# kurtosis/mat_mul

Hardware: NVIDIA B200
Metric: env_steps_per_sec (higher is better)
Workload: dtype int8

## Files before the change

mat_mul_b200/csrc/tg_demo.cu:

```cuda
#include <cstring>
#include <mutex>

#include "tg_demo_mma.cuh"
#include "tg_demo_sampler.cuh"
#include "tg_step.cuh"

namespace tg {

template <int S, int NT, int NPASS = 1>
struct DemoCfg {
    using G = Geo<S>;
    static constexpr int GPASS = NT / S;
    static constexpr int TG = GPASS * NPASS;
    static constexpr int ACTIVE = GPASS * S;
    static constexpr bool TILE = S != 4;
    static constexpr int KW = (S + 3) / 4;
    static constexpr int NCW = (2 * S + 3) / 4;
    static constexpr int NW = (3 * S + 3) / 4;
    static constexpr int REC = G::TP;
    static_assert(4 * (KW + NCW) <= REC, "record does not fit the token pitch");
    static constexpr int PITCH = G::GP + (S == 9 ? 32 : (S == 4 ? 16 : 0));
    static constexpr int PASS_SLAB = TILE ? GPASS * PITCH : 0;
    static __host__ __device__ constexpr int rec_bytes(int R) { return R * TG * REC; }
    static __host__ __device__ constexpr int rec_region(int R) { return (rec_bytes(R) + 15) & ~15; }
    static constexpr bool SPLIT = S == 9;
    static constexpr int REC_SMEM = SPLIT ? 36 : REC;
    static __host__ __device__ constexpr int pass_rec(int R) { return GPASS * R * REC_SMEM; }
    static __host__ __device__ constexpr int pass_stride(int R) { return ((pass_rec(R) > PASS_SLAB ? pass_rec(R) : PASS_SLAB) + 15) & ~15; }
    static __host__ __device__ constexpr int main_bytes(int R) { return NPASS * pass_stride(R); }
    static __device__ __forceinline__ void rec_pos(int g, int r, int R, int &region, int &k) {
        const int pass = NPASS == 1 ? 0 : g / GPASS;
        region = pass * pass_stride(R), k = (g - pass * GPASS) * R + r;
    }
    static __device__ __forceinline__ int slab_off(int g, int R) {
        if constexpr (NPASS == 1) return g * PITCH;
        const int pass = g / GPASS;
        return pass * pass_stride(R) + (g - pass * GPASS) * PITCH;
    }
    static constexpr int FLAG_BYTES = ((TG + 3) & ~3) * 4;
    static __host__ __device__ constexpr int smem_bytes(int R) { return main_bytes(R) + FLAG_BYTES + 16 + 2 * NT * 4; }
};

template <int S, int NT, int NPASS, bool SMALL>
__device__ __forceinline__ void emit_record(const uint32_t words[(3 * S + 3) / 4], int shift, uint8_t *region, int k, int R) {
    using C = DemoCfg<S, NT, NPASS>;
    constexpr int o = 2 * S;
    constexpr uint32_t WLAST = (S % 4) ? (0xFFFFFFFFu >> (8 * (4 - S % 4))) : 0xFFFFFFFFu;
    const uint32_t sh4 = (uint32_t)shift * ONES4;
    uint32_t out[C::REC / 4];
#pragma unroll
    for (int m = 0; m < C::REC / 4; m++) out[m] = 0;
#pragma unroll
    for (int m = 0; m < C::KW; m++) {
        const uint32_t lo = words[(o >> 2) + m];
        uint32_t wt = lo;
        if constexpr ((o & 3) != 0) {
            const uint32_t hi = ((o >> 2) + m + 1 < C::NW) ? words[(o >> 2) + m + 1] : 0u;
            wt = __funnelshift_r(lo, hi, 8 * (o & 3));
        }
        const uint32_t msk = (m == C::KW - 1) ? WLAST : 0xFFFFFFFFu;
        out[m] = (wt & msk) - (sh4 & msk);
    }
#pragma unroll
    for (int m = 0; m < C::NCW; m++) out[C::KW + m] = SMALL ? (words[m] + (H4 - sh4)) ^ H4 : ((words[m] | H4) - sh4) ^ H4;
    if constexpr (C::SPLIT) {
        static_assert(!C::SPLIT || (C::KW == 3 && C::NCW == 5), "split records: 9x9x9");
        const int n = C::GPASS * R;
        *reinterpret_cast<uint4 *>(region + k * 16) = make_uint4(out[0], out[1], out[2], out[3]);
        *reinterpret_cast<uint2 *>(region + n * 16 + k * 8) = make_uint2(out[4], out[5]);
        uint32_t *v = reinterpret_cast<uint32_t *>(region + n * 24 + k * 12);
        v[0] = out[5], v[1] = out[6], v[2] = out[7];
    } else {
        static_assert(C::REC % 16 == 0, "record pitch");
        uint8_t *rec = region + k * C::REC;
#pragma unroll
        for (int m = 0; m < C::REC / 16; m++)
            reinterpret_cast<uint4 *>(rec)[m] = make_uint4(out[4 * m], out[4 * m + 1], out[4 * m + 2], out[4 * m + 3]);
    }
}

template <int B>
__device__ __forceinline__ int coef_byte(uint32_t w) {
    constexpr uint32_t sel = (uint32_t)B | ((uint32_t)(B | 8) << 4) | ((uint32_t)(B | 8) << 8) | ((uint32_t)(B | 8) << 12);
    return (int)prmt(w, 0u, sel);
}

template <int S, int NT, int NPASS, bool SAMPLE, int NTHR, bool GUARD, int MMA = 0, bool ALIAS = false>
__global__ void __launch_bounds__(NT, S == 16 ? (NT <= 128 ? 4 : 2) : (S == 9 ? (NT == 128 ? 8 : NT == 64 ? 16 : 3) : 4))
    demo_kernel(unsigned long long first_demo, long long N, int R, uint32_t magic_r, int shift,
                const __grid_constant__ Categorical cat, int max_tries, uint8_t *__restrict__ tape,
                long long tape_step_stride, int8_t *__restrict__ slab, uint8_t *__restrict__ flags,
                const __grid_constant__ AliasDev ap) {
    using C = DemoCfg<S, NT, NPASS>;
    using G = Geo<S>;
    extern __shared__ __align__(128) uint8_t smem[];
    uint8_t *s_rec = smem;
    constexpr int MMA_SCRATCH = MMA > 0 ? (NT / 32) * acc16::WARP_WORDS * 4 : 0;
    uint32_t *s_flag = reinterpret_cast<uint32_t *>(smem + (MMA == 0 ? C::main_bytes(R) : MMA > 0 ? C::rec_region(R) + MMA_SCRATCH : 0));
    uint32_t *s_work = s_flag + C::FLAG_BYTES / 4;
    uint32_t *s_list = s_work + 4;
    uint32_t *s_alias = MMA > 0 ? reinterpret_cast<uint32_t *>(smem + C::rec_region(R)) : s_list;

    const int tid = threadIdx.x;
    const int lane = tid & 31;
    const long long g0 = (long long)blockIdx.x * C::TG;
    const int ng = (int)min((long long)C::TG, N - g0);
    const int npairs = ng * R;

    for (int g = tid; g < C::TG; g += NT) s_flag[g] = 0;
    if (tid < 3) s_work[tid] = 0;
    if constexpr (ALIAS) alias_to_smem<S, NT>(ap, s_alias);
    __syncthreads();

    if constexpr (SAMPLE && ALIAS) {
        for (int p = tid; p < npairs; p += NT) {
            const int g = magic_r ? (int)__umulhi((uint32_t)p, magic_r) : p;
            const int r = p - g * R;
            const unsigned long long d = first_demo + (unsigned long long)(g0 + g);
            uint32_t words[G::TP / 4];
#pragma unroll
            for (int w = C::NW; w < G::TP / 4; w++) words[w] = 0;
            draw_triple_alias<S>(words, (uint32_t)d, (uint32_t)(d >> 32), r, ap, s_alias);
            uint4 *dst = reinterpret_cast<uint4 *>(tape + (size_t)r * tape_step_stride + (g0 + g) * G::TP);
#pragma unroll
            for (int w = 0; w < G::TP / 16; w++) dst[w] = make_uint4(words[4 * w], words[4 * w + 1], words[4 * w + 2], words[4 * w + 3]);
            if constexpr (MMA == 0) {
                {
                    int region, k;
                    C::rec_pos(g, r, R, region, k);
                    emit_record<S, NT, NPASS, true>(words, shift, smem + region, k, R);
                }
            } else if constexpr (MMA > 0) {
                uint4 *rdst = reinterpret_cast<uint4 *>(s_rec + ((size_t)g * R + r) * G::TP);
#pragma unroll
                for (int w = 0; w < G::TP / 16; w++) rdst[w] = make_uint4(words[4 * w], words[4 * w + 1], words[4 * w + 2], words[4 * w + 3]);
            }
        }
    } else if constexpr (SAMPLE) {
        auto decode = [&](int p, int &g, int &r, uint32_t &d_lo, uint32_t &d_hi) {
            g = magic_r ? (int)__umulhi((uint32_t)p, magic_r) : p;
            r = p - g * R;
            const unsigned long long d = first_demo + (unsigned long long)(g0 + g);
            d_lo = (uint32_t)d, d_hi = (uint32_t)(d >> 32);
        };
        auto attempt = [&](int g, int r, uint32_t d_lo, uint32_t d_hi, int t) -> bool {
            uint32_t words[G::TP / 4];
#pragma unroll
            for (int w = C::NW; w < G::TP / 4; w++) words[w] = 0;
            bool ok = draw_triple<S, NTHR>(words, d_lo, d_hi, r, t, cat);
            if (!ok && t + 1 >= max_tries) {
#pragma unroll
                for (int w = 0; w < C::NW; w++) words[w] = 0;
#pragma unroll
                for (int q = 0; q < 3 * S; q++)
                    words[q >> 2] |= (((q % S) == 0 ? cat.top_tok : (uint32_t)shift) & 0xFFu) << (8 * (q & 3));
                atomicOr(&s_flag[g], (uint32_t)TG_FLAG_EXHAUSTED);
                ok = true;
            }
            if (ok) {
                uint4 *dst = reinterpret_cast<uint4 *>(tape + (size_t)r * tape_step_stride + (g0 + g) * G::TP);
#pragma unroll
                for (int w = 0; w < G::TP / 16; w++)
                    dst[w] = make_uint4(words[4 * w], words[4 * w + 1], words[4 * w + 2], words[4 * w + 3]);
                if constexpr (MMA == 0) {
                    {
                    int region, k;
                    C::rec_pos(g, r, R, region, k);
                    emit_record<S, NT, NPASS, false>(words, shift, smem + region, k, R);
                }
                } else if constexpr (MMA > 0) {
                    uint4 *rdst = reinterpret_cast<uint4 *>(s_rec + ((size_t)g * R + r) * G::TP);
#pragma unroll
                    for (int w = 0; w < G::TP / 16; w++)
                        rdst[w] = make_uint4(words[4 * w], words[4 * w + 1], words[4 * w + 2], words[4 * w + 3]);
                }
            }
            return ok;
        };
        auto park = [&](bool pending, int p, int t, int which) {
            const uint32_t m = __ballot_sync(0xFFFFFFFFu, pending);
            if (m) {
                const int leader = __ffs(m) - 1;
                int base = 0;
                if (lane == leader) base = (int)atomicAdd(&s_work[1 + which], (uint32_t)__popc(m));
                base = __shfl_sync(0xFFFFFFFFu, base, leader);
                if (pending) s_list[which * NT + base + __popc(m & ((1u << lane) - 1u))] = (uint32_t)p | ((uint32_t)t << 16);
            }
        };
        {
            int p = npairs, t = 0, g = 0, r = 0;
            uint32_t d_lo = 0, d_hi = 0;
            bool need = true;
            while (true) {
                const uint32_t m = __ballot_sync(0xFFFFFFFFu, need);
                if (m) {
                    const int leader = __ffs(m) - 1;
                    int base = 0;
                    if (lane == leader) base = (int)atomicAdd(&s_work[0], (uint32_t)__popc(m));
                    base = __shfl_sync(0xFFFFFFFFu, base, leader);
                    if (need) {
                        p = base + __popc(m & ((1u << lane) - 1u));
                        t = 0, need = false;
                        if (p < npairs) decode(p, g, r, d_lo, d_hi);
                    }
                }
                if (__ballot_sync(0xFFFFFFFFu, p >= npairs) != 0) {
                    park(p < npairs, p, t, 0);
                    break;
                }
                if (attempt(g, r, d_lo, d_hi, t))
                    need = true;
                else
                    t++;
            }
        }
        __syncthreads();
        for (int cur = 0;; cur ^= 1) {
            const int n = (int)s_work[1 + cur];
            if (n == 0) break;
            __syncthreads();
            if (tid == 0) s_work[1 + (cur ^ 1)] = 0;
            __syncthreads();
            const bool have = tid < n;
            int p = 0, t = 0, g = 0, r = 0;
            uint32_t d_lo = 0, d_hi = 0;
            bool pending = false;
            if (have) {
                const uint32_t it = s_list[cur * NT + tid];
                p = (int)(it & 0xFFFFu), t = (int)(it >> 16);
                decode(p, g, r, d_lo, d_hi);
                pending = true;
            }
#pragma unroll 1
            for (int k = 0; k < 3; k++) {
                if (pending) {
                    pending = !attempt(g, r, d_lo, d_hi, t);
                    t++;
                }
                if (__ballot_sync(0xFFFFFFFFu, pending) == 0) break;
            }
            park(pending, p, t, cur ^ 1);
            __syncthreads();
        }
    } else {
        for (int p = tid; p < npairs; p += NT) {
            const int g = magic_r ? (int)__umulhi((uint32_t)p, magic_r) : p;
            const int r = p - g * R;
            const uint4 *src = reinterpret_cast<const uint4 *>(tape + (size_t)r * tape_step_stride + (g0 + g) * G::TP);
            uint32_t words[G::TP / 4];
#pragma unroll
            for (int w = 0; w < G::TP / 16; w++) {
                const uint4 q = src[w];
                words[4 * w] = q.x, words[4 * w + 1] = q.y, words[4 * w + 2] = q.z, words[4 * w + 3] = q.w;
            }
            {
                    int region, k;
                    C::rec_pos(g, r, R, region, k);
                    emit_record<S, NT, NPASS, false>(words, shift, smem + region, k, R);
                }
        }
    }
    __syncthreads();
    if constexpr (MMA != 0) {
        if constexpr (MMA > 0) {
            static_assert(MMA <= 0 || (S == 16 && G::TP == 48), "tensor-core accumulation: 16x16x16 only");
            const int warp = tid >> 5;
            uint32_t *sH = reinterpret_cast<uint32_t *>(smem + C::rec_region(R)) + warp * acc16::WARP_WORDS, *sU = sH + acc16::H_WORDS;
            for (int g = warp; g < ng; g += NT / 32) {
#pragma unroll
                for (int pass = 0; pass < (MMA + 1) / 2; pass++) {
                    const int r = 32 * pass + lane;
                    if (r < 16 * MMA) {
                        const uint32_t z = (uint32_t)shift * ONES4;
                        uint4 raw[3] = {make_uint4(z, z, z, z), make_uint4(z, z, z, z), make_uint4(z, z, z, z)};
                        if (r < R) {
                            const uint4 *src = reinterpret_cast<const uint4 *>(s_rec + ((size_t)g * R + r) * G::TP);
                            raw[0] = src[0], raw[1] = src[1], raw[2] = src[2];
                        }
                        acc16::record_to_halves(raw, shift, sH + r * acc16::HP);
                    }
                }
                __syncwarp();
                const bool bad = acc16::gemms_from_halves<MMA>(sH, sU, slab + (g0 + g) * G::GP, lane);
                if (bad && lane == 0) s_flag[g] |= (uint32_t)TG_FLAG_RANGE;
            }
            __syncthreads();
        }
        if (flags)
            for (int gg = tid; gg < ng; gg += NT) flags[g0 + gg] = (uint8_t)s_flag[gg];
        return;
    }

    constexpr int KW = C::KW;
    const bool sparse = cat.sparse_terms && R <= 32;
#pragma unroll 1
    for (int pass = 0; pass < NPASS; pass++) {
    int gl = tid / S, j = tid % S;
    bool worker = tid < C::ACTIVE && pass * C::GPASS + gl < ng;
    uint32_t tmask = 0;
    if (sparse) {
        if (worker) {
            const uint8_t *region = smem + pass * C::pass_stride(R);
            const int8_t *vb = reinterpret_cast<const int8_t *>(
                C::SPLIT ? region + C::GPASS * R * 24 + gl * R * 12 + 1 + j : region + gl * R * C::REC + 4 * C::KW + S + j);
            uint32_t bit = 1;
#pragma unroll 4
            for (int r = 0; r < R; r++, bit <<= 1)
                if (vb[r * (C::SPLIT ? 12 : C::REC)] != 0) tmask |= bit;
        }
    }
    const int g = pass * C::GPASS + gl;
// ... 243 lines not shown
    }
    const int warp = threadIdx.x >> 5, lane = threadIdx.x & 31;
    const long long nw0 = (long long)blockIdx.x * 128 + warp * 32;
    if (nw0 >= N) return;
    const bool real = nw0 + lane < N;
    const long long n = min(nw0 + lane, N - 1);
    const unsigned long long d = first_demo + (unsigned long long)n;
    uint32_t acc[16];
#pragma unroll
    for (int e = 0; e < 16; e++) acc[e] = H4;
    const uint32_t sh4 = (uint32_t)shift * ONES4;
    uint4 *rec = reinterpret_cast<uint4 *>(tape + n * 16);
    const long long stride16 = tape_step_stride / 16;
    uint4 nextq = (!SAMPLE && R > 0) ? __ldg(reinterpret_cast<const uint4 *>(rec)) : make_uint4(0, 0, 0, 0);
    for (int r = 0; r < R; r++) {
        uint32_t words[3];
        uint32_t cu, cv;
        if constexpr (SAMPLE) {
            draw_triple_alias<S>(words, (uint32_t)d, (uint32_t)(d >> 32), r, ap, s_alias);
            if (real) rec[(long long)r * stride16] = make_uint4(words[0], words[1], words[2], 0u);
            cu = (words[0] + (H4 - sh4)) ^ H4, cv = (words[1] + (H4 - sh4)) ^ H4;
        } else {
            words[0] = nextq.x, words[1] = nextq.y, words[2] = nextq.z;
            if (r + 1 < R) nextq = __ldg(reinterpret_cast<const uint4 *>(rec) + (long long)(r + 1) * stride16);
            cu = ((words[0] | H4) - sh4) ^ H4, cv = ((words[1] | H4) - sh4) ^ H4;
        }
        const int wi = (int)(words[2] - sh4);
        const int vw[4] = {coef_byte<0>(cv) * wi, coef_byte<1>(cv) * wi, coef_byte<2>(cv) * wi, coef_byte<3>(cv) * wi};
        const int u[4] = {coef_byte<0>(cu), coef_byte<1>(cu), coef_byte<2>(cu), coef_byte<3>(cu)};
#pragma unroll
        for (int i = 0; i < 4; i++)
#pragma unroll
            for (int j = 0; j < 4; j++) acc[4 * i + j] += (uint32_t)(u[i] * vw[j]);
    }
    uint32_t ok = H4;
    uint4 *mine = reinterpret_cast<uint4 *>(s_stage[warp] + lane * PITCH);
#pragma unroll
    for (int i = 0; i < 4; i++) {
#pragma unroll
        for (int j = 0; j < 4; j++) {
            const uint32_t o = acc[4 * i + j];
            ok &= o ^ (o << 1);
            acc[4 * i + j] = o ^ H4;
        }
        mine[i] = make_uint4(acc[4 * i], acc[4 * i + 1], acc[4 * i + 2], acc[4 * i + 3]);
    }
    if (flags && real) flags[n] = (~ok & H4) ? (uint8_t)TG_FLAG_RANGE : (uint8_t)0;
    __syncwarp();
    const int total = (int)min(32LL, N - nw0) * 4;
    uint4 *out = reinterpret_cast<uint4 *>(slab + nw0 * 64);
    for (int x = lane; x < total; x += 32) out[x] = *reinterpret_cast<const uint4 *>(s_stage[warp] + (x >> 2) * PITCH + (x & 3) * 16);
}

static int dispatch_demo_alias(unsigned long long first, long long N, int R, int S, int shift, const Categorical &cat,
                               const AliasDev &ap, uint8_t *tape, long long stride, int8_t *slab, uint8_t *flags, cudaStream_t st) {
    switch (S) {
    case 4:
#ifdef TG_TUNING
        if (tuning_env("TG_DEMO_VARIANT", 0) == 0)
#endif
        if ((long long)R * shift * shift * shift <= 191 && R <= 65535) {
            const long long grid = (N + 127) / 128;
            if (grid > 0x7FFFFFFFLL) return TG_E_ARG;
            demo4_thread_kernel<true><<<(int)grid, 128, 0, st>>>(first, N, R, shift, tape, stride, slab, flags, ap);
            TG_CUDA(cudaGetLastError());
            return TG_OK;
        }
        if (DemoCfg<4, 256, 4>::smem_bytes(R) <= 160 * 1024)
            return launch_demo_alias<4, 256, 4, 0>(first, N, R, shift, cat, ap, tape, stride, slab, flags, st);
        return launch_demo_alias<4, 256, 1, 0>(first, N, R, shift, cat, ap, tape, stride, slab, flags, st);
    case 9:
#ifdef TG_TUNING
        switch (tuning_env("TG_DEMO_VARIANT", 0)) {
        case 1: return launch_demo_alias<9, 256, 1, 0>(first, N, R, shift, cat, ap, tape, stride, slab, flags, st);
        case 2: return launch_demo_alias<9, 128, 1, 0>(first, N, R, shift, cat, ap, tape, stride, slab, flags, st);
        case 3: return launch_demo_alias<9, 256, 2, 0>(first, N, R, shift, cat, ap, tape, stride, slab, flags, st);
        case 4: return launch_demo_alias<9, 64, 2, 0>(first, N, R, shift, cat, ap, tape, stride, slab, flags, st);
        case 5: return launch_demo_alias<9, 64, 1, 0>(first, N, R, shift, cat, ap, tape, stride, slab, flags, st);
        default: break;
        }
#endif
        return launch_demo_alias<9, 128, 2, 0>(first, N, R, shift, cat, ap, tape, stride, slab, flags, st);
    case 16:
        if (demo_acc16_mma_applies(R)) {
            if (R <= 32) return launch_demo_alias<16, 128, 2, 2>(first, N, R, shift, cat, ap, tape, stride, slab, flags, st);
            return launch_demo_alias<16, 128, 2, 4>(first, N, R, shift, cat, ap, tape, stride, slab, flags, st);
        }
        return launch_demo_alias<16, 128, 1, 0>(first, N, R, shift, cat, ap, tape, stride, slab, flags, st);
    }
    return TG_E_ARG;
}

constexpr int ALIAS_SLOTS = 8, ALIAS_MAXDEV = 64;
__device__ __align__(16) uint32_t g_alias_tab[ALIAS_SLOTS][8 * ALIAS_BUCKETS];
__global__ void alias_upload_kernel(const __grid_constant__ AliasTabs t, int slot) {
    for (int w = threadIdx.x; w < 8 * ALIAS_BUCKETS; w += blockDim.x) g_alias_tab[slot][w] = (&t.tab[0][0])[w];
}
struct AliasSlot {
    bool valid = false;
    AliasTabs host;
    cudaEvent_t ready = nullptr;
    unsigned long long stamp = 0;
};
static AliasSlot g_alias_slots[ALIAS_MAXDEV][ALIAS_SLOTS];
static std::mutex g_alias_mu;
static unsigned long long g_alias_stamp = 0;

int alias_device_tables(const AliasTabs &want, cudaStream_t st, const uint32_t **dptr) {
    int dev = 0;
    TG_CUDA(cudaGetDevice(&dev));
    if (dev < 0 || dev >= ALIAS_MAXDEV) return TG_E_ARG;
    uint32_t *base = nullptr;
    TG_CUDA(cudaGetSymbolAddress(reinterpret_cast<void **>(&base), g_alias_tab));
    std::lock_guard<std::mutex> lock(g_alias_mu);
    AliasSlot *slots = g_alias_slots[dev];
    int hit = -1, lru = -1;
    for (int i = 0; i < ALIAS_SLOTS; i++) {
        if (slots[i].valid && memcmp(&slots[i].host, &want, sizeof(AliasTabs)) == 0) hit = i;
        if (lru < 0 || (slots[lru].valid && (!slots[i].valid || slots[i].stamp < slots[lru].stamp))) lru = i;
    }
    if (hit < 0) {
        AliasSlot &sl = slots[lru];
        if (sl.valid) TG_CUDA(cudaDeviceSynchronize());
        if (!sl.ready) TG_CUDA(cudaEventCreateWithFlags(&sl.ready, cudaEventDisableTiming));
        sl.valid = false;
        alias_upload_kernel<<<1, 256, 0, st>>>(want, lru);
        TG_CUDA(cudaGetLastError());
        TG_CUDA(cudaEventRecord(sl.ready, st));
        sl.host = want, sl.valid = true;
        hit = lru;
    } else {
        TG_CUDA(cudaStreamWaitEvent(st, slots[hit].ready, 0));
    }
    slots[hit].stamp = ++g_alias_stamp;
    *dptr = base + (size_t)hit * 8 * ALIAS_BUCKETS;
// ... 76 lines not shown
    }
    __syncthreads();
    if (flags && tid == 0) flags[n] = (uint8_t)((or_flags ? flags[n] : 0) | s_bad);
}

template <int S>
static int launch_demo_acc_cols(const uint8_t *tape, long long stride, long long N, int R, int shift, int8_t *slab, uint8_t *flags,
                                int or_flags, cudaStream_t st) {
    const long long smem = (long long)R * Geo<S>::TP;
    if (smem > 227 * 1024 || N > 0x7FFFFFFFLL) return TG_E_ARG;
    auto kern = demo_acc_cols_kernel<S>;
    TG_CUDA(cudaFuncSetAttribute(kern, cudaFuncAttributeMaxDynamicSharedMemorySize, (int)smem));
    kern<<<(unsigned)N, 160, (size_t)smem, st>>>(tape, stride, N, R, shift, slab, flags, or_flags);
    TG_CUDA(cudaGetLastError());
    return TG_OK;
}

template <int NTHR>
static int launch_demo25(unsigned long long first, long long N, int R, int shift, const Categorical &cat, int max_tries, uint8_t *tape,
                         long long stride, int8_t *slab, uint8_t *flags, cudaStream_t st) {
    constexpr int NT = 128;
    using C = DemoCfg<25, NT, 1>;
    const int smem = C::FLAG_BYTES + 16 + 2 * NT * 4;
    if (R > 65535 || (long long)C::TG * R >= (1LL << 16)) return TG_E_ARG;
    const uint32_t magic = R == 1 ? 0u : (uint32_t)((0x100000000ULL + (unsigned)R - 1) / (unsigned)R);
    const long long grid = (N + C::TG - 1) / C::TG;
    if (grid > 0x7FFFFFFFLL) return TG_E_ARG;
    static const AliasDev no_alias = {};
    demo_kernel<25, NT, 1, true, NTHR, false, -1><<<(int)grid, NT, smem, st>>>(first, N, R, magic, shift, cat, max_tries, tape, stride,
                                                                              nullptr, flags, no_alias);
    TG_CUDA(cudaGetLastError());
    return launch_demo_acc_cols<25>(tape, stride, N, R, shift, slab, flags, 1, st);
}

template <bool SAMPLE, int NTHR>
static int dispatch_demo(unsigned long long first, long long N, int R, int S, int shift, const Categorical &cat,
                         int max_tries, uint8_t *tape, long long stride, int8_t *slab, uint8_t *flags, cudaStream_t st) {
    switch (S) {
    case 4: {
#ifdef TG_TUNING
        static const int variant = tuning_env("TG_DEMO_VARIANT", 0);
        if (variant == 1 && DemoCfg<4, 128, 8>::smem_bytes(R) <= 160 * 1024)
            return launch_demo<4, 128, 8, SAMPLE, NTHR>(first, N, R, shift, cat, max_tries, tape, stride, slab, flags, st);
        if (variant == 2 && DemoCfg<4, 128, 4>::smem_bytes(R) <= 160 * 1024)
            return launch_demo<4, 128, 4, SAMPLE, NTHR>(first, N, R, shift, cat, max_tries, tape, stride, slab, flags, st);
        if (variant == 3 && DemoCfg<4, 512, 2>::smem_bytes(R) <= 160 * 1024)
            return launch_demo<4, 512, 2, SAMPLE, NTHR>(first, N, R, shift, cat, max_tries, tape, stride, slab, flags, st);
#endif
        if (DemoCfg<4, 256, 4>::smem_bytes(R) <= 160 * 1024)
            return launch_demo<4, 256, 4, SAMPLE, NTHR>(first, N, R, shift, cat, max_tries, tape, stride, slab, flags, st);
        return launch_demo<4, 256, 1, SAMPLE, NTHR>(first, N, R, shift, cat, max_tries, tape, stride, slab, flags, st);
    }
    case 9: {
#ifdef TG_TUNING
        switch (tuning_env("TG_DEMO_VARIANT", 0)) {
        case 1: return launch_demo<9, 256, 1, SAMPLE, NTHR>(first, N, R, shift, cat, max_tries, tape, stride, slab, flags, st);
        case 3: return launch_demo<9, 128, 3, SAMPLE, NTHR>(first, N, R, shift, cat, max_tries, tape, stride, slab, flags, st);
        case 4: return launch_demo<9, 192, 2, SAMPLE, NTHR>(first, N, R, shift, cat, max_tries, tape, stride, slab, flags, st);
        case 5: return launch_demo<9, 64, 4, SAMPLE, NTHR>(first, N, R, shift, cat, max_tries, tape, stride, slab, flags, st);
        default: break;
        }
#endif
        if (SAMPLE) return launch_demo<9, 128, 2, SAMPLE, NTHR>(first, N, R, shift, cat, max_tries, tape, stride, slab, flags, st);
        return launch_demo<9, 128, 1, SAMPLE, NTHR>(first, N, R, shift, cat, max_tries, tape, stride, slab, flags, st);
    }
    case 16: {
#ifdef TG_TUNING
        static const int variant = tuning_env("TG_DEMO_VARIANT", 0);
        if (variant == 1) return launch_demo<16, 256, 1, SAMPLE, NTHR>(first, N, R, shift, cat, max_tries, tape, stride, slab, flags, st);
        if (variant == 2) return launch_demo<16, 64, 1, SAMPLE, NTHR>(first, N, R, shift, cat, max_tries, tape, stride, slab, flags, st);
        if (variant == 3) return launch_demo<16, 128, 2, SAMPLE, NTHR>(first, N, R, shift, cat, max_tries, tape, stride, slab, flags, st);
#endif
        return launch_demo<16, 128, 1, SAMPLE, NTHR>(first, N, R, shift, cat, max_tries, tape, stride, slab, flags, st);
    }
    }
    return TG_E_ARG;
}

}

extern "C" {

int tg_demo_gen_philox(uint64_t seed, uint64_t first_demo, int64_t N, int R, int S, int shift, const int8_t *values,
                       const double *probs, int n_values, int max_tries, uint8_t *tape, int64_t tape_step_stride,
                       int8_t *slab, uint8_t *flags, void *stream) {
    if (!tg::supported_S(S) || N < 0 || R < 1 || shift < 1 || shift > 4 || n_values < 1 || n_values > 8 || max_tries < 1 ||
        max_tries > 65535)
        return TG_E_ARG;
    if (N == 0) return TG_OK;
    if (!values || !probs || !tape || !slab) return TG_E_ARG;
    if (((uintptr_t)tape | (uintptr_t)slab | (uintptr_t)tape_step_stride) & 15) return TG_E_ARG;
    if (!tg::alphabet_ok(values, probs, n_values, shift)) return TG_E_ARG;
    tg::Categorical cat = tg::categorical(values, probs, n_values, shift, seed);
    cat.sparse_terms = (S == 9 && tg::p_null<false>(values, probs, n_values) >= 0.5) ? 1u : 0u;
    cudaStream_t st = (cudaStream_t)stream;
    if (tg::alias_applies(values, probs, n_values, S)) {
        tg::AliasParams ap;
        tg::build_alias(values, probs, n_values, S, shift, seed, ap);
        tg::AliasTabs tabs;
        tg::AliasDev dev;
        tg::alias_to_dev(ap, values, n_values, S, shift, tabs, dev);
        const int rc = tg::alias_device_tables(tabs, st, &dev.tab);
        if (rc != TG_OK) return rc;
        return tg::dispatch_demo_alias(first_demo, N, R, S, shift, cat, dev, tape, tape_step_stride, slab, flags, st);
    }
#ifdef TG_TUNING
    static const int use_mma = tg::tuning_env("TG_DEMO_MMA", 1);
#else
    constexpr int use_mma = 1;
#endif
    if (S == 25) {
        if (n_values <= 3) return tg::launch_demo25<2>(first_demo, N, R, shift, cat, max_tries, tape, tape_step_stride, slab, flags, st);
        if (n_values <= 5) return tg::launch_demo25<4>(first_demo, N, R, shift, cat, max_tries, tape, tape_step_stride, slab, flags, st);
        return tg::launch_demo25<7>(first_demo, N, R, shift, cat, max_tries, tape, tape_step_stride, slab, flags, st);
    }
    if (S == 16 && use_mma && tg::demo_acc16_mma_applies(R)) {
        if (n_values <= 3) return tg::dispatch_demo16_mma<2>(first_demo, N, R, shift, cat, max_tries, tape, tape_step_stride, slab, flags, st);
        if (n_values <= 5) return tg::dispatch_demo16_mma<4>(first_demo, N, R, shift, cat, max_tries, tape, tape_step_stride, slab, flags, st);
        return tg::dispatch_demo16_mma<7>(first_demo, N, R, shift, cat, max_tries, tape, tape_step_stride, slab, flags, st);
    }
    if (n_values <= 3)
        return tg::dispatch_demo<true, 2>(first_demo, N, R, S, shift, cat, max_tries, tape, tape_step_stride, slab, flags, st);
    if (n_values <= 5)
        return tg::dispatch_demo<true, 4>(first_demo, N, R, S, shift, cat, max_tries, tape, tape_step_stride, slab, flags, st);
    return tg::dispatch_demo<true, 7>(first_demo, N, R, S, shift, cat, max_tries, tape, tape_step_stride, slab, flags, st);
}

int tg_demo_alias_tables(const int8_t *values, const double *probs, int n_values, int S, uint16_t *tables_host) {
    if (!values || !probs || !tables_host || !tg::alias_applies(values, probs, n_values, S)) return TG_E_ARG;
    tg::AliasParams ap;
    tg::build_alias(values, probs, n_values, S, 0, 0, ap);
    memcpy(tables_host, ap.tab[6], sizeof(ap.tab[6]));
    memcpy(tables_host + tg::ALIAS_BUCKETS, ap.tab[7], sizeof(ap.tab[7]));
    memcpy(tables_host + 2 * tg::ALIAS_BUCKETS, ap.tab[0], 6 * sizeof(ap.tab[0]));
    return TG_OK;
}

int tg_demo_accumulate(const uint8_t *tape, int64_t tape_step_stride, int64_t N, int R, int S, int shift, int8_t *slab,
                       uint8_t *flags, void *stream) {
    if (!tg::supported_S(S) || N < 0 || R < 1 || shift < 1 || shift > 4) return TG_E_ARG;
    if (N == 0) return TG_OK;
    if (!tape || !slab) return TG_E_ARG;
    if (((uintptr_t)tape | (uintptr_t)slab | (uintptr_t)tape_step_stride) & 15) return TG_E_ARG;
#ifdef TG_TUNING
    static const int use_mma = tg::tuning_env("TG_DEMO_MMA", 1);
#else
    constexpr int use_mma = 1;
#endif
    if (S == 25) return tg::launch_demo_acc_cols<25>(tape, tape_step_stride, N, R, shift, slab, flags, 0, (cudaStream_t)stream);
    if (S == 16 && use_mma && tg::demo_acc16_mma_applies(R))
        return tg::launch_demo_acc16_mma(tape, tape_step_stride, N, R, shift, slab, flags, 0, (cudaStream_t)stream);
    if (S == 4 && (long long)R * shift * shift * shift <= 191 && R <= 65535 && N <= 0x7FFFFFFFLL * 128) {
        static const tg::AliasDev no_tables = {};
        tg::demo4_thread_kernel<false><<<(int)((N + 127) / 128), 128, 0, (cudaStream_t)stream>>>(0, N, R, shift, const_cast<uint8_t *>(tape),
                                                                                              tape_step_stride, slab, flags, no_tables);
        TG_CUDA(cudaGetLastError());
        return TG_OK;
    }
    tg::Categorical cat = {};
    cat.sparse_terms = S == 9 ? 1u : 0u;
    return tg::dispatch_demo<false, 2>(0, N, R, S, shift, cat, 1, const_cast<uint8_t *>(tape), tape_step_stride, slab, flags,
                                       (cudaStream_t)stream);
}

}
```

Before: 4.172 billion.

## Add dedicated single-pass S=9 demo kernel for alias sampling and accumulation

Adds a specialised demo9_kernel for 9x9x9 that samples (or reads) tape tokens, emits split records into shared memory, and has each of the 9 threads per game accumulate one output column before bulk-copying the finished tile to global memory. Threads in a group count completion with a shared atomic, so the last one issues the bulk store and writes the flag without a block-wide pass. The alias-sampling and non-sampling S=9 paths are routed to this kernel, and emit_record is decoupled from the NT/NPASS config. It raises shared-memory use per block and relies on per-group atomics plus proxy fences for correctness.

```diff
diff --git a/mat_mul_b200/csrc/tg_demo.cu b/mat_mul_b200/csrc/tg_demo.cu
--- a/mat_mul_b200/csrc/tg_demo.cu
+++ b/mat_mul_b200/csrc/tg_demo.cu
@@ -41,9 +41,9 @@
     static __host__ __device__ constexpr int smem_bytes(int R) { return main_bytes(R) + FLAG_BYTES + 16 + 2 * NT * 4; }
 };
 
-template <int S, int NT, int NPASS, bool SMALL>
-__device__ __forceinline__ void emit_record(const uint32_t words[(3 * S + 3) / 4], int shift, uint8_t *region, int k, int R) {
-    using C = DemoCfg<S, NT, NPASS>;
+template <int S, bool SMALL>
+__device__ __forceinline__ void emit_record(const uint32_t words[(3 * S + 3) / 4], int shift, uint8_t *region, int k, int n) {
+    using C = DemoCfg<S, 32>;
     constexpr int o = 2 * S;
     constexpr uint32_t WLAST = (S % 4) ? (0xFFFFFFFFu >> (8 * (4 - S % 4))) : 0xFFFFFFFFu;
     const uint32_t sh4 = (uint32_t)shift * ONES4;
@@ -65,7 +65,6 @@
     for (int m = 0; m < C::NCW; m++) out[C::KW + m] = SMALL ? (words[m] + (H4 - sh4)) ^ H4 : ((words[m] | H4) - sh4) ^ H4;
     if constexpr (C::SPLIT) {
         static_assert(!C::SPLIT || (C::KW == 3 && C::NCW == 5), "split records: 9x9x9");
-        const int n = C::GPASS * R;
         *reinterpret_cast<uint4 *>(region + k * 16) = make_uint4(out[0], out[1], out[2], out[3]);
         *reinterpret_cast<uint2 *>(region + n * 16 + k * 8) = make_uint2(out[4], out[5]);
         uint32_t *v = reinterpret_cast<uint32_t *>(region + n * 24 + k * 12);
@@ -128,7 +127,7 @@
                 {
                     int region, k;
                     C::rec_pos(g, r, R, region, k);
-                    emit_record<S, NT, NPASS, true>(words, shift, smem + region, k, R);
+                    emit_record<S, true>(words, shift, smem + region, k, C::GPASS * R);
                 }
             } else if constexpr (MMA > 0) {
                 uint4 *rdst = reinterpret_cast<uint4 *>(s_rec + ((size_t)g * R + r) * G::TP);
@@ -166,7 +165,7 @@
                     {
                     int region, k;
                     C::rec_pos(g, r, R, region, k);
-                    emit_record<S, NT, NPASS, false>(words, shift, smem + region, k, R);
+                    emit_record<S, false>(words, shift, smem + region, k, C::GPASS * R);
                 }
                 } else if constexpr (MMA > 0) {
                     uint4 *rdst = reinterpret_cast<uint4 *>(s_rec + ((size_t)g * R + r) * G::TP);
@@ -256,7 +255,7 @@
             {
                     int region, k;
                     C::rec_pos(g, r, R, region, k);
-                    emit_record<S, NT, NPASS, false>(words, shift, smem + region, k, R);
+                    emit_record<S, false>(words, shift, smem + region, k, C::GPASS * R);
                 }
         }
     }
@@ -606,6 +605,212 @@
     for (int x = lane; x < total; x += 32) out[x] = *reinterpret_cast<const uint4 *>(s_stage[warp] + (x >> 2) * PITCH + (x & 3) * 16);
 }
 
+template <int NT>
+struct Demo9Cfg {
+    using G = Geo<9>;
+    static constexpr int TG = NT / 9;
+    static constexpr int PITCH = DemoCfg<9, NT>::PITCH;
+    static constexpr int TILE_BYTES = TG * PITCH;
+    static __host__ __device__ constexpr int rec_bytes(int R) { return (TG * R * 36 + 15) & ~15; }
+    static __host__ __device__ constexpr int cnt_off(int R, bool sample) { return TILE_BYTES + rec_bytes(R) + (sample ? AliasGeo<9>::SMEM_BYTES : 0); }
+    static __host__ __device__ constexpr int smem_bytes(int R, bool sample) { return cnt_off(R, sample) + TG * 4; }
+};
+
+template <int NT, bool SAMPLE, bool GUARD>
+__global__ void __launch_bounds__(NT, 1024 / NT)
+    demo9_kernel(unsigned long long first_demo, long long N, int R, int shift, int sparse_terms,
+                 uint8_t *__restrict__ tape, long long tape_step_stride, int8_t *__restrict__ slab, uint8_t *__restrict__ flags,
+                 const __grid_constant__ AliasDev ap) {
+    constexpr int S = 9, KW = 3;
+    using C = Demo9Cfg<NT>;
+    using G = Geo<S>;
+    constexpr int TG = C::TG;
+    extern __shared__ __align__(128) uint8_t smem[];
+    uint8_t *s_tile = smem, *s_rec = smem + C::TILE_BYTES;
+    uint32_t *s_alias = reinterpret_cast<uint32_t *>(smem + C::TILE_BYTES + C::rec_bytes(R));
+    uint32_t *s_cnt = reinterpret_cast<uint32_t *>(smem + C::cnt_off(R, SAMPLE));
+
+    const int tid = threadIdx.x;
+    const long long g0 = (long long)blockIdx.x * TG;
+    const int ng = (int)min((long long)TG, N - g0);
+    const int nrec = TG * R;
+
+    for (int x = tid; x < TG * 12; x += NT) {
+        const int g = x / 12, w = x - 12 * g;
+        *reinterpret_cast<uint32_t *>(s_tile + g * C::PITCH + (w < 9 ? w * G::RP + 80 : S * G::RP + 4 * (w - 9))) = 0u;
+    }
+    for (int g = tid; g < TG; g += NT) s_cnt[g] = 0;
+    if constexpr (SAMPLE) {
+        alias_to_smem<S, NT>(ap, s_alias);
+        __syncthreads();
+    }
+
+    for (int p = tid; p < nrec; p += NT) {
+        const int r = p / TG, g = p - r * TG;
+        if (g >= ng) continue;
+        uint32_t words[G::TP / 4];
+        uint4 *tp = reinterpret_cast<uint4 *>(tape + (size_t)r * tape_step_stride + (g0 + g) * G::TP);
+        if constexpr (SAMPLE) {
+            const unsigned long long d = first_demo + (unsigned long long)(g0 + g);
+#pragma unroll
+            for (int w = DemoCfg<S, NT>::NW; w < G::TP / 4; w++) words[w] = 0;
+            draw_triple_alias<S>(words, (uint32_t)d, (uint32_t)(d >> 32), r, ap, s_alias);
+#pragma unroll
+            for (int w = 0; w < G::TP / 16; w++) tp[w] = make_uint4(words[4 * w], words[4 * w + 1], words[4 * w + 2], words[4 * w + 3]);
+        } else {
+#pragma unroll
+            for (int w = 0; w < G::TP / 16; w++) {
+                const uint4 q = tp[w];
+                words[4 * w] = q.x, words[4 * w + 1] = q.y, words[4 * w + 2] = q.z, words[4 * w + 3] = q.w;
+            }
+        }
+        emit_record<S, SAMPLE>(words, shift, s_rec, g * R + r, nrec);
+    }
+    __syncthreads();
+
+    const int g = tid / S, j = tid - g * S;
+    if (g >= ng) return;
+    const uint8_t *rx = s_rec + g * R * 16, *ry = s_rec + nrec * 16 + g * R * 8;
+    const int8_t *rv = reinterpret_cast<const int8_t *>(s_rec + nrec * 24 + 1) + g * R * 12 + j;
+    const bool sparse = sparse_terms && R <= 32;
+    uint32_t tmask = 0;
+    if (sparse) {
+#pragma unroll 4
+        for (int r = 0; r < R; r++)
+            if (rv[r * 12] != 0) tmask |= 1u << r;
+    }
+    int32_t acc[S][KW];
+#pragma unroll
+    for (int i = 0; i < S; i++)
+#pragma unroll
+        for (int m = 0; m < KW; m++) acc[i][m] = (int32_t)H4;
+    int bound = 0;
+    auto term = [&](int r) {
+        const uint4 xq = *reinterpret_cast<const uint4 *>(rx + r * 16);
+        const uint2 yq = *reinterpret_cast<const uint2 *>(ry + r * 8);
+        const int vj = (int)rv[r * 12];
+        if constexpr (GUARD) bound += abs(vj);
+        const int32_t vw[KW] = {vj * (int32_t)xq.x, vj * (int32_t)xq.y, vj * (int32_t)xq.z};
+        const uint32_t cu[3] = {xq.w, yq.x, yq.y};
+#pragma unroll
+        for (int i = 0; i < S; i++) {
+            const uint32_t b = i & 3;
+            const int ui = (int)prmt(cu[i >> 2], 0u, b | ((b | 8) << 4) | ((b | 8) << 8) | ((b | 8) << 12));
+#pragma unroll
+            for (int m = 0; m < KW; m++) acc[i][m] += ui * vw[m];
+        }
+    };
+    if (sparse) {
+        while (tmask) {
+            const int t = 31 - __clz((int)tmask);
+            tmask ^= 1u << t;
+            term(t);
+        }
+    } else {
+#pragma unroll 2
+        for (int r = 0; r < R; r++) term(r);
+    }
+    uint32_t bad = 0;
+    if (GUARD && bound * shift * shift > 191) {
+#pragma unroll
+        for (int i = 0; i < S; i++)
+#pragma unroll
+            for (int m = 0; m < KW; m++) {
+                uint32_t word = 0;
+#pragma unroll 1
+                for (int kk = 0; kk < 4; kk++) {
+                    const int k = 4 * m + kk;
+                    if (k >= S) break;
+                    int e = 0;
+#pragma unroll 1
+                    for (int r = 0; r < R; r++) {
+                        const uint32_t w = reinterpret_cast<const uint32_t *>(rx + r * 16)[m];
+                        const uint32_t cu = i < 4 ? reinterpret_cast<const uint32_t *>(rx + r * 16)[3]
+                                                  : reinterpret_cast<const uint32_t *>(ry + r * 8)[(i - 4) >> 2];
+                        const uint32_t wb = (w + H4) ^ H4;
+                        const int ui = (int)(int8_t)((cu >> (8 * (i & 3))) & 0xFFu);
+                        e += ui * (int)rv[r * 12] * (int)(int8_t)((wb >> (8 * kk)) & 0xFFu);
+                    }
+                    if (e < -64 || e > 63) bad = 1;
+                    word |= ((uint32_t)e & 0xFFu) << (8 * kk);
+                }
+                acc[i][m] = (int32_t)word;
+            }
+    } else {
+        uint32_t ok = H4;
+#pragma unroll
+        for (int i = 0; i < S; i++)
+#pragma unroll
+            for (int m = 0; m < KW; m++) {
+                const uint32_t o = (uint32_t)acc[i][m];
+                ok &= o ^ (o << 1);
+                acc[i][m] = (int32_t)(o ^ H4);
+            }
+        bad = ~ok & H4;
+    }
+    uint8_t *gbase = s_tile + g * C::PITCH + j * S;
+    const int sj = j & 1;
+#pragma unroll
+    for (int i = 0; i < S; i++) {
+        const uint32_t w0 = (uint32_t)acc[i][0], w1 = (uint32_t)acc[i][1], w2 = (uint32_t)acc[i][2];
+        const uint32_t x0 = __funnelshift_r(w0, w1, 8 * sj), x1 = __funnelshift_r(w1, w2, 8 * sj);
+        uint8_t *rowp = gbase + i * G::RP;
+        uint16_t *hp = reinterpret_cast<uint16_t *>(rowp + sj);
+        hp[0] = (uint16_t)x0, hp[1] = (uint16_t)(x0 >> 16), hp[2] = (uint16_t)x1, hp[3] = (uint16_t)(x1 >> 16);
+        rowp[sj ? 0 : 8] = (uint8_t)(sj ? w0 : w2);
+    }
+    fence_proxy_async();
+    __threadfence_block();
+    const uint32_t add = 1u | (bad ? 0x100u << j : 0u);
+    const uint32_t done = atomicAdd(&s_cnt[g], add) + add;
+    if ((done & 0xFFu) == S) {
+        __threadfence_block();
+        fence_proxy_async();
+        bulk_s2g(slab + (g0 + g) * G::GP, s_tile + g * C::PITCH, (uint32_t)G::GP);
+        bulk_commit();
+        if (flags) flags[g0 + g] = (done >> 8) ? (uint8_t)TG_FLAG_RANGE : (uint8_t)0;
+        bulk_wait<0>();
+    }
+}
+
+template <int NT, bool SAMPLE>
+static int launch_demo9(unsigned long long first, long long N, int R, int shift, bool sparse, const AliasDev &ap, uint8_t *tape,
+                        long long stride, int8_t *slab, uint8_t *flags, cudaStream_t st) {
+    using C = Demo9Cfg<NT>;
+    const int smem = C::smem_bytes(R, SAMPLE);
+    if (smem > 227 * 1024 || R > 65535 || (long long)C::TG * R >= (1LL << 16)) return TG_E_ARG;
+    const long long grid = (N + C::TG - 1) / C::TG;
+    if (grid > 0x7FFFFFFFLL) return TG_E_ARG;
+    if ((long long)R * shift * shift * shift > 191) {
+        auto kern = demo9_kernel<NT, SAMPLE, true>;
+        TG_CUDA(cudaFuncSetAttribute(kern, cudaFuncAttributeMaxDynamicSharedMemorySize, smem));
+        kern<<<(int)grid, NT, smem, st>>>(first, N, R, shift, sparse, tape, stride, slab, flags, ap);
+    } else {
+        auto kern = demo9_kernel<NT, SAMPLE, false>;
+        TG_CUDA(cudaFuncSetAttribute(kern, cudaFuncAttributeMaxDynamicSharedMemorySize, smem));
+        kern<<<(int)grid, NT, smem, st>>>(first, N, R, shift, sparse, tape, stride, slab, flags, ap);
+    }
+    TG_CUDA(cudaGetLastError());
+    return TG_OK;
+}
+
+template <bool SAMPLE>
+static int dispatch_demo9(unsigned long long first, long long N, int R, int shift, bool sparse, const AliasDev &ap, uint8_t *tape,
+                          long long stride, int8_t *slab, uint8_t *flags, cudaStream_t st) {
+#ifdef TG_TUNING
+    switch (tuning_env("TG_DEMO_VARIANT", 0)) {
+    case 1: return launch_demo9<128, SAMPLE>(first, N, R, shift, sparse, ap, tape, stride, slab, flags, st);
+    case 2: return launch_demo9<256, SAMPLE>(first, N, R, shift, sparse, ap, tape, stride, slab, flags, st);
+    default: break;
+    }
+#endif
+    if (SAMPLE && Demo9Cfg<256>::smem_bytes(R, SAMPLE) <= 227 * 1024)
+        return launch_demo9<256, SAMPLE>(first, N, R, shift, sparse, ap, tape, stride, slab, flags, st);
+    if (Demo9Cfg<128>::smem_bytes(R, SAMPLE) <= 227 * 1024)
+        return launch_demo9<128, SAMPLE>(first, N, R, shift, sparse, ap, tape, stride, slab, flags, st);
+    return launch_demo9<64, SAMPLE>(first, N, R, shift, sparse, ap, tape, stride, slab, flags, st);
+}
+
 static int dispatch_demo_alias(unsigned long long first, long long N, int R, int S, int shift, const Categorical &cat,
                                const AliasDev &ap, uint8_t *tape, long long stride, int8_t *slab, uint8_t *flags, cudaStream_t st) {
     switch (S) {
@@ -624,17 +829,7 @@
             return launch_demo_alias<4, 256, 4, 0>(first, N, R, shift, cat, ap, tape, stride, slab, flags, st);
         return launch_demo_alias<4, 256, 1, 0>(first, N, R, shift, cat, ap, tape, stride, slab, flags, st);
     case 9:
-#ifdef TG_TUNING
-        switch (tuning_env("TG_DEMO_VARIANT", 0)) {
-        case 1: return launch_demo_alias<9, 256, 1, 0>(first, N, R, shift, cat, ap, tape, stride, slab, flags, st);
-        case 2: return launch_demo_alias<9, 128, 1, 0>(first, N, R, shift, cat, ap, tape, stride, slab, flags, st);
-        case 3: return launch_demo_alias<9, 256, 2, 0>(first, N, R, shift, cat, ap, tape, stride, slab, flags, st);
-        case 4: return launch_demo_alias<9, 64, 2, 0>(first, N, R, shift, cat, ap, tape, stride, slab, flags, st);
-        case 5: return launch_demo_alias<9, 64, 1, 0>(first, N, R, shift, cat, ap, tape, stride, slab, flags, st);
-        default: break;
-        }
-#endif
-        return launch_demo_alias<9, 128, 2, 0>(first, N, R, shift, cat, ap, tape, stride, slab, flags, st);
+        return dispatch_demo9<true>(first, N, R, shift, cat.sparse_terms != 0, ap, tape, stride, slab, flags, st);
     case 16:
         if (demo_acc16_mma_applies(R)) {
             if (R <= 32) return launch_demo_alias<16, 128, 2, 2>(first, N, R, shift, cat, ap, tape, stride, slab, flags, st);
@@ -817,6 +1012,7 @@
         return launch_demo<4, 256, 1, SAMPLE, NTHR>(first, N, R, shift, cat, max_tries, tape, stride, slab, flags, st);
     }
     case 9: {
+        if constexpr (!SAMPLE) return TG_E_ARG;
 #ifdef TG_TUNING
         switch (tuning_env("TG_DEMO_VARIANT", 0)) {
         case 1: return launch_demo<9, 256, 1, SAMPLE, NTHR>(first, N, R, shift, cat, max_tries, tape, stride, slab, flags, st);
@@ -826,8 +1022,7 @@
         default: break;
         }
 #endif
-        if (SAMPLE) return launch_demo<9, 128, 2, SAMPLE, NTHR>(first, N, R, shift, cat, max_tries, tape, stride, slab, flags, st);
-        return launch_demo<9, 128, 1, SAMPLE, NTHR>(first, N, R, shift, cat, max_tries, tape, stride, slab, flags, st);
+        return launch_demo<9, 128, 2, SAMPLE, NTHR>(first, N, R, shift, cat, max_tries, tape, stride, slab, flags, st);
     }
     case 16: {
 #ifdef TG_TUNING
@@ -922,8 +1117,12 @@
         TG_CUDA(cudaGetLastError());
         return TG_OK;
     }
+    if (S == 9) {
+        static const tg::AliasDev no_tables = {};
+        return tg::dispatch_demo9<false>(0, N, R, shift, true, no_tables, const_cast<uint8_t *>(tape), tape_step_stride, slab, flags,
+                                         (cudaStream_t)stream);
+    }
     tg::Categorical cat = {};
-    cat.sparse_terms = S == 9 ? 1u : 0u;
     return tg::dispatch_demo<false, 2>(0, N, R, S, shift, cat, 1, const_cast<uint8_t *>(tape), tape_step_stride, slab, flags,
                                        (cudaStream_t)stream);
 }
```

New measurement: 4.178 billion, median of 6. About the same (+0.1%).

## Add row-owner warp kernel for 9x9x9 demo generation with sparse term ordering

Applied to the files above, without the earlier changes.

Adds a new demo9_rows_kernel in which each warp handles 7 games and each lane owns one output row, accumulating rank-R products in packed SWAR registers. Sparse inputs are reordered by popcount so lanes with similar term counts run together. The kernel replaces the previous tiled alias and replay paths as the default for S=9. This is meant to improve parallelism and cut tile overhead, but it adds per-lane work imbalance, extra shared-memory staging, and a guarded slow path for range overflow.

```diff
diff --git a/mat_mul_b200/csrc/tg_demo.cu b/mat_mul_b200/csrc/tg_demo.cu
--- a/mat_mul_b200/csrc/tg_demo.cu
+++ b/mat_mul_b200/csrc/tg_demo.cu
@@ -3,6 +3,7 @@
 
 #include "tg_demo_mma.cuh"
 #include "tg_demo_sampler.cuh"
+#include "tg_rows.cuh"
 #include "tg_step.cuh"
 
 namespace tg {
@@ -606,6 +607,274 @@
     for (int x = lane; x < total; x += 32) out[x] = *reinterpret_cast<const uint4 *>(s_stage[warp] + (x >> 2) * PITCH + (x & 3) * 16);
 }
 
+struct Demo9Rows {
+    static constexpr int W = 7;
+    static constexpr int GPITCH = 784;
+    static __host__ __device__ constexpr int a16(int x) { return (x + 15) & ~15; }
+    static __host__ __device__ constexpr int y_off(int R) { return a16(W * R * 16); }
+    static __host__ __device__ constexpr int u_off(int R) { return y_off(R) + a16(W * R * 8); }
+    static __host__ __device__ constexpr int stage_off(int R) { return u_off(R) + a16(W * R * 12); }
+    static __host__ __device__ constexpr int mask_off(int R, bool st) { return stage_off(R) + (st ? W * GPITCH : 0); }
+    static __host__ __device__ constexpr int order_off(int R, bool st) { return mask_off(R, st) + 64 * 4; }
+    static __host__ __device__ constexpr int hist_off(int R, bool st) { return order_off(R, st) + 64; }
+    static __host__ __device__ constexpr int flag_off(int R, bool st) { return hist_off(R, st) + 32 * 4; }
+    static __host__ __device__ constexpr int jm_off(int R, bool st) { return flag_off(R, st) + 8 * 4; }
+    static __host__ __device__ constexpr int warp_bytes(int R, bool st) { return jm_off(R, st) + 8 * 4; }
+    template <bool SAMPLE, bool STAGE>
+    static __host__ __device__ constexpr long long smem_bytes(int NT, int R) {
+        return (SAMPLE ? a16(AliasGeo<9>::SMEM_BYTES) : 0) + (long long)(NT / 32) * warp_bytes(R, STAGE);
+    }
+};
+static_assert(Demo9Rows::W * 9 <= 64 && Demo9Rows::W <= 8 && Demo9Rows::GPITCH % 16 == 0, "row-owner demo geometry");
+
+template <bool SMALL>
+__device__ __forceinline__ void emit_record9_rows(const uint32_t words[7], int shift, uint8_t *sx, uint8_t *sy, uint8_t *su, int k) {
+    const uint32_t sh4 = (uint32_t)shift * ONES4;
+    uint32_t c[5];
+#pragma unroll
+    for (int m = 0; m < 5; m++) c[m] = SMALL ? (words[m] + (H4 - sh4)) ^ H4 : ((words[m] | H4) - sh4) ^ H4;
+    const uint32_t w0 = __funnelshift_r(words[4], words[5], 16) - sh4;
+    const uint32_t w1 = __funnelshift_r(words[5], words[6], 16) - sh4;
+    const uint32_t w2 = (__funnelshift_r(words[6], 0u, 16) & 0xFFu) - (sh4 & 0xFFu);
+    *reinterpret_cast<uint4 *>(sx + k * 16) = make_uint4(w0, w1, w2, __funnelshift_r(c[2], c[3], 8));
+    *reinterpret_cast<uint2 *>(sy + k * 8) = make_uint2(__funnelshift_r(c[3], c[4], 8), (c[4] >> 8) & 0xFFu);
+    uint32_t *u = reinterpret_cast<uint32_t *>(su + k * 12);
+    u[0] = c[0], u[1] = c[1], u[2] = c[2] & 0xFFu;
+}
+
+template <int NT, bool SAMPLE, bool GUARD, bool STAGE>
+__global__ void __launch_bounds__(NT, NT == 128 ? (STAGE ? 4 : 8) : 8)
+    demo9_rows_kernel(unsigned long long first_demo, long long N, int R, uint32_t magic_r, int shift, int sparse,
+                      uint8_t *__restrict__ tape, long long tape_step_stride, int8_t *__restrict__ slab,
+                      uint8_t *__restrict__ flags, const __grid_constant__ AliasDev ap) {
+    using D = Demo9Rows;
+    using G = Geo<9>;
+    constexpr int S = 9, W = D::W;
+    extern __shared__ __align__(128) uint8_t smem[];
+    constexpr int TAB = SAMPLE ? D::a16(AliasGeo<S>::SMEM_BYTES) : 0;
+    if constexpr (SAMPLE) {
+        alias_to_smem<S, NT>(ap, reinterpret_cast<uint32_t *>(smem));
+        __syncthreads();
+    }
+    const int warp = threadIdx.x >> 5, lane = threadIdx.x & 31;
+    const long long gw0 = ((long long)blockIdx.x * (NT / 32) + warp) * W;
+    if (gw0 >= N) return;
+    const int nw = (int)min((long long)W, N - gw0), nrows = 9 * nw;
+    uint8_t *base = smem + TAB + warp * D::warp_bytes(R, STAGE);
+    uint8_t *sx = base, *sy = base + D::y_off(R), *su = base + D::u_off(R), *stage = base + D::stage_off(R);
+    uint32_t *s_mask = reinterpret_cast<uint32_t *>(base + D::mask_off(R, STAGE));
+    uint8_t *s_order = base + D::order_off(R, STAGE);
+    uint32_t *s_hist = reinterpret_cast<uint32_t *>(base + D::hist_off(R, STAGE));
+    uint32_t *s_flag = reinterpret_cast<uint32_t *>(base + D::flag_off(R, STAGE));
+    uint32_t *s_jm = reinterpret_cast<uint32_t *>(base + D::jm_off(R, STAGE));
+    if (lane < 8) s_flag[lane] = 0, s_jm[lane] = 0;
+    s_hist[lane] = 0;
+
+    for (int p = lane; p < nw * R; p += 32) {
+        const int g = magic_r ? (int)__umulhi((uint32_t)p, magic_r) : p;
+        const int r = p - g * R;
+        uint32_t words[G::TP / 4];
+        uint4 *t = reinterpret_cast<uint4 *>(tape + (size_t)r * tape_step_stride + (gw0 + g) * G::TP);
+        if constexpr (SAMPLE) {
+            const unsigned long long d = first_demo + (unsigned long long)(gw0 + g);
+#pragma unroll
+            for (int w = (3 * S + 3) / 4; w < G::TP / 4; w++) words[w] = 0;
+            draw_triple_alias<S>(words, (uint32_t)d, (uint32_t)(d >> 32), r, ap, reinterpret_cast<const uint32_t *>(smem));
+#pragma unroll
+            for (int w = 0; w < G::TP / 16; w++) t[w] = make_uint4(words[4 * w], words[4 * w + 1], words[4 * w + 2], words[4 * w + 3]);
+        } else {
+#pragma unroll
+            for (int w = 0; w < G::TP / 16; w++) {
+                const uint4 q = t[w];
+                words[4 * w] = q.x, words[4 * w + 1] = q.y, words[4 * w + 2] = q.z, words[4 * w + 3] = q.w;
+            }
+        }
+        emit_record9_rows<SAMPLE>(words, shift, sx, sy, su, p);
+    }
+    __syncwarp();
+
+    uint32_t tm[2] = {0u, 0u};
+#pragma unroll
+    for (int h = 0; h < 2; h++) {
+        const int n = lane + 32 * h;
+        if (n < nrows) {
+            const int g = n / 9, i = n - 9 * g, k0 = g * R;
+            if (sparse) {
+                const int8_t *ub = reinterpret_cast<const int8_t *>(su + k0 * 12 + i);
+#pragma unroll 4
+                for (int r = 0; r < R; r++)
+                    if (ub[r * 12] != 0) tm[h] |= 1u << r;
+            }
+            if constexpr (GUARD) {
+                const int8_t *vb = reinterpret_cast<const int8_t *>(i < 4 ? sx + k0 * 16 + 12 + i : sy + k0 * 8 + (i - 4));
+                const int pitch = i < 4 ? 16 : 8;
+                int bound = 0;
+#pragma unroll 1
+                for (int r = 0; r < R; r++) bound += abs((int)vb[r * pitch]);
+                if (bound * shift * shift > 191) atomicOr(&s_jm[g], 1u << i);
+            }
+            s_mask[n] = tm[h];
+        }
+    }
+    if (sparse) {
+        int key[2], pos[2];
+#pragma unroll
+        for (int h = 0; h < 2; h++) {
+            key[h] = min(__popc(tm[h]), 31);
+            pos[h] = lane + 32 * h < nrows ? (int)atomicAdd(&s_hist[key[h]], 1u) : 0;
+        }
+        __syncwarp();
+        const int cnt = (int)s_hist[lane];
+        int incl = cnt;
+#pragma unroll
+        for (int o = 1; o < 32; o <<= 1) {
+            const int x = __shfl_up_sync(0xFFFFFFFFu, incl, o);
+            if (lane >= o) incl += x;
+        }
+#pragma unroll
+        for (int h = 0; h < 2; h++) {
+            const int b = __shfl_sync(0xFFFFFFFFu, incl - cnt, key[h]);
+            if (lane + 32 * h < nrows) s_order[b + pos[h]] = (uint8_t)(lane + 32 * h);
+        }
+    }
+    __syncwarp();
+
+#pragma unroll 1
+    for (int c0 = 0; c0 < nrows; c0 += 32) {
+        const bool act = c0 + lane < nrows;
+        const int n = !act ? 0 : sparse ? (int)s_order[c0 + lane] : c0 + lane;
+        const int g = n / 9, i = n - 9 * g, k0 = g * R;
+        const uint8_t *rx = sx + k0 * 16, *ry = sy + k0 * 8;
+        const int8_t *ru = reinterpret_cast<const int8_t *>(su + k0 * 12 + i);
+        uint32_t run[9][3];
+#pragma unroll
+        for (int j = 0; j < 9; j++)
+#pragma unroll
+            for (int m = 0; m < 3; m++) run[j][m] = H4;
+        auto term = [&](int t) {
+            const uint4 x = *reinterpret_cast<const uint4 *>(rx + t * 16);
+            const uint2 y = *reinterpret_cast<const uint2 *>(ry + t * 8);
+            const uint32_t u = (uint32_t)(int)ru[t * 12];
+            const uint32_t uw[3] = {u * x.x, u * x.y, u * x.z};
+            const int v[9] = {coef_byte<0>(x.w), coef_byte<1>(x.w), coef_byte<2>(x.w), coef_byte<3>(x.w),
+                              coef_byte<0>(y.x), coef_byte<1>(y.x), coef_byte<2>(y.x), coef_byte<3>(y.x), coef_byte<0>(y.y)};
+#pragma unroll
+            for (int j = 0; j < 9; j++)
+#pragma unroll
+                for (int m = 0; m < 3; m++) run[j][m] += (uint32_t)v[j] * uw[m];
+        };
+        if (sparse) {
+            uint32_t mask = act ? s_mask[n] : 0u;
+            while (mask) {
+                const int t = 31 - __clz((int)mask);
+                mask ^= 1u << t;
+                term(t);
+            }
+        } else if (act) {
+#pragma unroll 2
+            for (int r = 0; r < R; r++) term(r);
+        }
+        uint32_t ok = H4, bad = 0;
+        const uint32_t jm = GUARD && act ? s_jm[g] : 0u;
+#pragma unroll
+        for (int j = 0; j < 9; j++) {
+            if (GUARD && ((jm >> j) & 1u)) {
+#pragma unroll
+                for (int m = 0; m < 3; m++) {
+                    uint32_t word = 0;
+#pragma unroll 1
+                    for (int kk = 0; kk < 4; kk++) {
+                        const int k = 4 * m + kk;
+                        if (k >= S) break;
+                        int e = 0;
+#pragma unroll 1
+                        for (int r = 0; r < R; r++) {
+                            const uint4 x = *reinterpret_cast<const uint4 *>(rx + r * 16);
+                            const uint2 y = *reinterpret_cast<const uint2 *>(ry + r * 8);
+                            const uint32_t wm = m == 0 ? x.x : m == 1 ? x.y : x.z;
+                            const uint32_t wb = (wm + H4) ^ H4;
+                            const uint32_t vw = j < 4 ? x.w : j < 8 ? y.x : y.y;
+                            const int vj = (int)(int8_t)((vw >> (8 * (j & 3))) & 0xFFu);
+                            e += (int)ru[r * 12] * vj * (int)(int8_t)((wb >> (8 * kk)) & 0xFFu);
+                        }
+                        if (e < -64 || e > 63) bad = 1;
+                        word |= ((uint32_t)e & 0xFFu) << (8 * kk);
+                    }
+                    run[j][m] = word;
+                }
+            } else {
+#pragma unroll
+                for (int m = 0; m < 3; m++) {
+                    const uint32_t o = run[j][m];
+                    ok &= o ^ (o << 1);
+                    run[j][m] = o ^ H4;
+                }
+            }
+        }
+        bad |= ~ok & H4;
+        if (act) {
+            uint32_t rw[RowRuns<S>::WR];
+            pack_row<S>(run, rw);
+            uint32_t *dst = reinterpret_cast<uint32_t *>(STAGE ? stage + g * D::GPITCH + i * G::RP : (uint8_t *)slab + (gw0 + g) * G::GP + i * G::RP);
+#pragma unroll
+            for (int w = 0; w < RowRuns<S>::WR; w++) dst[w] = rw[w];
+            if (!STAGE && i == S - 1) dst[RowRuns<S>::WR] = dst[RowRuns<S>::WR + 1] = dst[RowRuns<S>::WR + 2] = 0u;
+            if (bad) atomicOr(&s_flag[g], (uint32_t)TG_FLAG_RANGE);
+        }
+    }
+    __syncwarp();
+
+    constexpr int Q = G::GP / 16;
+    static_assert(G::GP - S * G::RP == 12 && S * G::RP % 16 == 4, "9x9x9: the last 16 bytes of a game are one row word + padding");
+    uint4 *out = reinterpret_cast<uint4 *>(slab + gw0 * G::GP);
+    for (int x = lane; STAGE && x < nw * Q; x += 32) {
+        const int g = x / Q, q = x - Q * g;
+        uint4 v = *reinterpret_cast<const uint4 *>(stage + g * D::GPITCH + q * 16);
+        if (q == Q - 1) v.y = v.z = v.w = 0u;
+        out[x] = v;
+    }
+    if (flags && lane < nw) flags[gw0 + lane] = (uint8_t)s_flag[lane];
+}
+
+template <int NT, bool SAMPLE, bool STAGE = true>
+static int launch_demo9_rows(unsigned long long first, long long N, int R, int shift, bool sparse, const AliasDev &ap, uint8_t *tape,
+                             long long stride, int8_t *slab, uint8_t *flags, cudaStream_t st) {
+    const long long smem = Demo9Rows::smem_bytes<SAMPLE, STAGE>(NT, R);
+    if (smem > 227 * 1024 || R > 65535) return TG_E_ARG;
+    const uint32_t magic = R == 1 ? 0u : (uint32_t)((0x100000000ULL + (unsigned)R - 1) / (unsigned)R);
+    constexpr int TG = NT / 32 * Demo9Rows::W;
+    const long long grid = (N + TG - 1) / TG;
+    if (grid > 0x7FFFFFFFLL) return TG_E_ARG;
+    const int sp = sparse && R <= 32;
+    if ((long long)R * shift * shift * shift > 191) {
+        auto kern = demo9_rows_kernel<NT, SAMPLE, true, STAGE>;
+        TG_CUDA(cudaFuncSetAttribute(kern, cudaFuncAttributeMaxDynamicSharedMemorySize, (int)smem));
+        kern<<<(int)grid, NT, (size_t)smem, st>>>(first, N, R, magic, shift, sp, tape, stride, slab, flags, ap);
+    } else {
+        auto kern = demo9_rows_kernel<NT, SAMPLE, false, STAGE>;
+        TG_CUDA(cudaFuncSetAttribute(kern, cudaFuncAttributeMaxDynamicSharedMemorySize, (int)smem));
+        kern<<<(int)grid, NT, (size_t)smem, st>>>(first, N, R, magic, shift, sp, tape, stride, slab, flags, ap);
+    }
+    TG_CUDA(cudaGetLastError());
+    return TG_OK;
+}
+
+template <bool SAMPLE>
+static int dispatch_demo9_rows(unsigned long long first, long long N, int R, int shift, bool sparse, const AliasDev &ap, uint8_t *tape,
+                               long long stride, int8_t *slab, uint8_t *flags, cudaStream_t st) {
+#ifdef TG_TUNING
+    if (tuning_env("TG_DEMO_VARIANT", 0) == 7)
+        return launch_demo9_rows<32, SAMPLE>(first, N, R, shift, sparse, ap, tape, stride, slab, flags, st);
+    if (tuning_env("TG_DEMO_VARIANT", 0) == 8)
+        return launch_demo9_rows<64, SAMPLE>(first, N, R, shift, sparse, ap, tape, stride, slab, flags, st);
+    if (tuning_env("TG_DEMO_VARIANT", 0) == 9)
+        return launch_demo9_rows<128, SAMPLE, false>(first, N, R, shift, sparse, ap, tape, stride, slab, flags, st);
+#endif
+    if (Demo9Rows::smem_bytes<SAMPLE, true>(128, R) <= 227 * 1024)
+        return launch_demo9_rows<128, SAMPLE>(first, N, R, shift, sparse, ap, tape, stride, slab, flags, st);
+    return launch_demo9_rows<32, SAMPLE>(first, N, R, shift, sparse, ap, tape, stride, slab, flags, st);
+}
+
 static int dispatch_demo_alias(unsigned long long first, long long N, int R, int S, int shift, const Categorical &cat,
                                const AliasDev &ap, uint8_t *tape, long long stride, int8_t *slab, uint8_t *flags, cudaStream_t st) {
     switch (S) {
@@ -631,10 +900,11 @@
         case 3: return launch_demo_alias<9, 256, 2, 0>(first, N, R, shift, cat, ap, tape, stride, slab, flags, st);
         case 4: return launch_demo_alias<9, 64, 2, 0>(first, N, R, shift, cat, ap, tape, stride, slab, flags, st);
         case 5: return launch_demo_alias<9, 64, 1, 0>(first, N, R, shift, cat, ap, tape, stride, slab, flags, st);
+        case 6: return launch_demo_alias<9, 128, 2, 0>(first, N, R, shift, cat, ap, tape, stride, slab, flags, st);
         default: break;
         }
 #endif
-        return launch_demo_alias<9, 128, 2, 0>(first, N, R, shift, cat, ap, tape, stride, slab, flags, st);
+        return dispatch_demo9_rows<true>(first, N, R, shift, cat.sparse_terms != 0, ap, tape, stride, slab, flags, st);
     case 16:
         if (demo_acc16_mma_applies(R)) {
             if (R <= 32) return launch_demo_alias<16, 128, 2, 2>(first, N, R, shift, cat, ap, tape, stride, slab, flags, st);
@@ -827,7 +1097,12 @@
         }
 #endif
         if (SAMPLE) return launch_demo<9, 128, 2, SAMPLE, NTHR>(first, N, R, shift, cat, max_tries, tape, stride, slab, flags, st);
-        return launch_demo<9, 128, 1, SAMPLE, NTHR>(first, N, R, shift, cat, max_tries, tape, stride, slab, flags, st);
+#ifdef TG_TUNING
+        if (tuning_env("TG_DEMO_VARIANT", 0) == 6)
+            return launch_demo<9, 128, 1, SAMPLE, NTHR>(first, N, R, shift, cat, max_tries, tape, stride, slab, flags, st);
+#endif
+        static const AliasDev no_tables = {};
+        return dispatch_demo9_rows<false>(0, N, R, shift, cat.sparse_terms != 0, no_tables, tape, stride, slab, flags, st);
     }
     case 16: {
 #ifdef TG_TUNING
```

Result: no change. 4.177 billion before, 4.172 billion after (median of 6 runs) (-0.1%).
